# davidbau/rewriting

Hardware: NVIDIA H100
Metric: StyleGAN2-256 images/sec (higher is better)
Workload: dtype bf16x3 (3-term split bf16 operands, fp32 accumulate; fp32 in/out)

## Files before the change

### rewriting_b200/csrc/upconv_tc.cu

```cuda
#include <cstring>

#include "../../include/rewriting_b200.h"
#include "rw_common.cuh"

namespace rw {

struct UpFusedParams {
  int B, Cin, Cout, H, W;
  const float* demod;
  const float* bias;
  const float* noise;
  long long noise_bstride;
  const float* noise_w;
  const float* k4;
  const float* next_scale;
  void* next_hi;
  void* next_lo;
  float* y_out;
  int act;
  int ncg, nbands, nitems;
  long long* debug_prof;
};

namespace {

constexpr int UM = 128;
constexpr int UNC = 16;
constexpr int UN = 9 * UNC;
constexpr int UBK = 32;
constexpr int UK = 16;
constexpr int kUStages = 5;
constexpr int kUThreads = 384;
constexpr int kUTmaWarp = 8;
constexpr uint32_t kUProducerRegs = 40;
constexpr uint32_t kUConsumerRegs = 232;
constexpr int kUABytes = UM * UBK * 2;
constexpr int kUBBytes = UN * UBK * 2;
constexpr int kUStageBytes = 2 * kUABytes + 2 * kUBBytes;
constexpr int kUMailFloats = 2 * 2 * 4 * 2 * 32;
constexpr int kUOutSlotBytes = 64 * 32;
constexpr int kUOutQuarterBytes = 2 * kUOutSlotBytes;
constexpr int kUOutStageBytes = 4 * kUOutQuarterBytes;
constexpr int kUXchgFloat2 = 9 * 2 * 32;
constexpr int kUXchgBytes = 8 * kUXchgFloat2 * 8;
constexpr int kUSmemTotal =
    kUStages * kUStageBytes + kUMailFloats * 4 + kUOutStageBytes + kUXchgBytes + 512 + 256;
static_assert(kUSmemTotal <= 232448, "upconv_fused: shared memory over the per-block limit");

struct UBarriers {
  uint64_t full[kUStages];
  uint64_t empty[kUStages];
};

__device__ __forceinline__ void tma_load_5d(void* smem_dst, const CUtensorMap* m, uint64_t* bar,
                                            int32_t c0, int32_t c1, int32_t c2, int32_t c3,
                                            int32_t c4) {
  asm volatile(
      "cp.async.bulk.tensor.5d.shared::cluster.global.mbarrier::complete_tx::bytes"
      " [%0], [%1, {%3, %4, %5, %6, %7}], [%2];\n" ::"r"(smem_u32(smem_dst)),
      "l"(reinterpret_cast<uint64_t>(m)), "r"(smem_u32(bar)), "r"(c0), "r"(c1), "r"(c2), "r"(c3),
      "r"(c4)
      : "memory");
}

__device__ __forceinline__ float2 f2add(float2 a, float2 b) {
  return make_float2(__fadd_rn(a.x, b.x), __fadd_rn(a.y, b.y));
}
__device__ __forceinline__ float2 f2mul(float2 a, float2 b) {
  return make_float2(__fmul_rn(a.x, b.x), __fmul_rn(a.y, b.y));
}
__device__ __forceinline__ float2 f2fma(float2 a, float2 b, float2 c) {
  return make_float2(__fmaf_rn(a.x, b.x, c.x), __fmaf_rn(a.y, b.y, c.y));
}
__device__ __forceinline__ void mbar_wait_relaxed(uint64_t* bar, uint32_t parity) {
  uint32_t spins = 0;
  while (!mbar_try_wait(bar, parity)) {
    __nanosleep(40);
    if (++spins > RW_SPIN_LIMIT) __trap();
  }
}

__device__ __forceinline__ void sts_v4(uint32_t a, float x, float y, float z, float w) {
  asm volatile("st.shared.v4.f32 [%0], {%1, %2, %3, %4};\n" ::"r"(a), "f"(x), "f"(y), "f"(z), "f"(w)
               : "memory");
}
__device__ __forceinline__ void lds_v4(uint32_t a, float& x, float& y, float& z, float& w) {
  asm volatile("ld.shared.v4.f32 {%0, %1, %2, %3}, [%4];\n"
               : "=f"(x), "=f"(y), "=f"(z), "=f"(w)
               : "r"(a)
               : "memory");
}

constexpr int kBarPair = 3;

struct UpItem {
  int bg, band, cg;
  int y_first, y_emit, y_end;
};

__device__ __forceinline__ UpItem decode_item(int item, const UpFusedParams& p) {
  UpItem it;
  it.cg = item % p.ncg;
  const int r = item / p.ncg;
  it.band = r % p.nbands;
  it.bg = r / p.nbands;
  const int ya = 1 + (it.band * p.H) / p.nbands;
  const int yb = 1 + ((it.band + 1) * p.H) / p.nbands;
  it.y_emit = ya;
  it.y_first = ya - 2 < 0 ? 0 : ya - 2;
  it.y_end = yb;
  return it;
}

template <bool PROF, bool NCHW>
__global__ void __launch_bounds__(kUThreads, 1)
upconv_fused_kernel(const __grid_constant__ CUtensorMap map_a_hi,
                    const __grid_constant__ CUtensorMap map_a_lo,
                    const __grid_constant__ CUtensorMap map_w_hi,
                    const __grid_constant__ CUtensorMap map_w_lo,
                    const __grid_constant__ CUtensorMap map_o_hi,
                    const __grid_constant__ CUtensorMap map_o_lo, const UpFusedParams p) {
  extern __shared__ uint8_t smem_raw[];
  uint8_t* smem = reinterpret_cast<uint8_t*>((reinterpret_cast<uintptr_t>(smem_raw) + 511) &
                                             ~static_cast<uintptr_t>(511));
  float* mail = reinterpret_cast<float*>(smem + kUStages * kUStageBytes);
  uint8_t* out_stage = smem + kUStages * kUStageBytes + kUMailFloats * 4;
  float2* xchg = reinterpret_cast<float2*>(out_stage + kUOutStageBytes);
  UBarriers* bars = reinterpret_cast<UBarriers*>(out_stage + kUOutStageBytes + kUXchgBytes);

  const int warp = __shfl_sync(0xffffffffu, static_cast<int>(threadIdx.x >> 5), 0);
  const int lane = threadIdx.x & 31;
  const int kb_count = p.Cin / UBK;
  const int G = UM / p.W;

  if (warp == kUTmaWarp && lane == 0) {
    tma_prefetch_desc(&map_a_hi);
    tma_prefetch_desc(&map_a_lo);
    tma_prefetch_desc(&map_w_hi);
    tma_prefetch_desc(&map_w_lo);
    tma_prefetch_desc(&map_o_hi);
    tma_prefetch_desc(&map_o_lo);
    for (int s = 0; s < kUStages; ++s) {
      mbar_init(&bars->full[s], 1);
      mbar_init(&bars->empty[s], 2);
    }
    fence_mbar_init();
  }
  __syncthreads();

  if (warp < kUTmaWarp) {
    setmaxnreg_inc<kUConsumerRegs>();
    const int wg = warp >> 2;
    const int q = warp >> 1;
    const int h = warp & 1;
    int stage = 0;
    uint32_t phase = 0;
    const int g = lane >> 2, c = lane & 3;
    const int W = p.W;
    const int T0 = q * 32 + 4 * g;
    const int x0 = T0 & (W - 1);
    const int img_in_tile = T0 / W;
    const int Ho = 2 * p.H, Wo = 2 * W;
    const bool first_x = (x0 == 0), last_x = (x0 + 4 == W);
    const bool cross = W > 32;
    const bool mail_l = cross && g == 0 && !first_x, mail_r = cross && g == 7 && !last_x;
    float kv[4], kh[4];
    {
      const float k00 = __ldg(p.k4 + 15);
#pragma unroll
      for (int a = 0; a < 4; ++a) {
        kv[a] = __ldg(p.k4 + 15 - a * 4);
        kh[a] = __ldg(p.k4 + 15 - a) / k00;
      }
    }
    const float nw = (!NCHW || (p.noise != nullptr && p.noise_w != nullptr)) ? __ldg(p.noise_w) : 0.f;
    uint32_t step = 0;
    constexpr uint32_t kMailBufBytes = 2 * 4 * 2 * 32 * 4;
    const uint32_t mail_s = smem_u32(mail) + h * (4 * 2 * 32 * 4) + c * 32;
    const uint32_t post_r = mail_s + (q * 2 + 1) * 128, post_l = mail_s + (q * 2 + 0) * 128;
    const uint32_t read_l = mail_s + ((q - 1) * 2 + 1) * 128, read_r = mail_s + ((q + 1) * 2 + 0) * 128;
    const uint32_t slot_s = smem_u32(out_stage) + q * kUOutQuarterBytes;
    uint32_t st_addr[2];
    {
      const int m = lane >> 3, gp = lane & 7;
      const int Wm = W < 32 ? W : 32;
      const int tl = 4 * gp + m;
      const int il = tl / W;
      const int xg = ((4 * gp) & (Wm - 1)) >> 2;
#pragma unroll
      for (int xi = 0; xi < 2; ++xi) {
        uint32_t a = slot_s + (((il * 8 + 2 * m + xi) * (Wm >> 2) + xg) << 5) + (h << 4);
        a ^= ((a >> 7) & 1u) << 4;
        st_addr[xi] = a;
      }
    }
    const CUtensorMap* omap = h ? &map_o_lo : &map_o_hi;
    const uint32_t my_slot = slot_s + h * kUOutSlotBytes;
    const int o_xg = ((32 * q) & (W - 1)) >> 2;
    const int o_img = (32 * q) / W;
    long long prof_acc[16] = {0, 0, 0, 0, 0, 0, 0, 0, 0, 0, 0, 0, 0, 0, 0, 0};

    for (int item = blockIdx.x; item < p.nitems; item += gridDim.x) {
      const UpItem it = decode_item(item, p);
      const int b0 = it.bg * G;
      const int b = b0 + img_in_tile;
      const bool img_ok = b < p.B;
      const int c0 = it.cg * UNC + h * 8 + 2 * c;
      const size_t chan_o = static_cast<size_t>(img_ok ? b : 0) * p.Cout + c0;
      float2 dm = make_float2(1.f, 1.f), bs = make_float2(0.f, 0.f), ns = make_float2(1.f, 1.f);
      if (!NCHW || p.demod != nullptr) dm = __ldg(reinterpret_cast<const float2*>(p.demod + chan_o));
      if (!NCHW || (p.act && p.bias != nullptr)) bs = __ldg(reinterpret_cast<const float2*>(p.bias + c0));
      if (!NCHW) ns = __ldg(reinterpret_cast<const float2*>(p.next_scale + chan_o));
      const bool has_noise = !NCHW || (p.noise != nullptr && p.noise_w != nullptr);
      float2 c20[4], c21[4], c22[4];
      float2 w0[2][4], w1[2][4], w2[2][4];
#pragma unroll
      for (int j = 0; j < 4; ++j) {
        c20[j] = c21[j] = c22[j] = make_float2(0.f, 0.f);
        w0[0][j] = w0[1][j] = w1[0][j] = w1[1][j] = w2[0][j] = w2[1][j] = make_float2(0.f, 0.f);
      }
      const float* nrow_base = p.noise + static_cast<size_t>(img_ok ? b : 0) * p.noise_bstride + 2 * x0;
      __nv_bfloat16* out_hi = static_cast<__nv_bfloat16*>(p.next_hi);
      __nv_bfloat16* out_lo = static_cast<__nv_bfloat16*>(p.next_lo);
      const size_t img_row0 = static_cast<size_t>(img_ok ? b : 0) * (Ho + 1);

      for (int y = it.y_first; y < it.y_end; ++y, ++step) {
        const bool rows_out = (y >= it.y_emit);
        const bool emit = rows_out && img_ok;
        if (emit && c < 2 && has_noise) {
          const float* np = nrow_base + static_cast<size_t>(2 * y - 2 + c) * Wo;
          asm volatile("prefetch.global.L1 [%0];\n" ::"l"(np));
        }
        long long tq[8];
        if constexpr (PROF) tq[0] = clock64();
        float2 P[9][4];
        {
          float d[72];
          int held = -1;
          for (int kb = 0; kb < kb_count; ++kb) {
            mbar_wait(&bars->full[stage], phase);
            const uint32_t sa = smem_u32(smem + stage * kUStageBytes);
            const uint64_t da_hi = make_smem_desc(sa + wg * (kUABytes / 2), 16, 512, 2);
            const uint64_t da_lo = make_smem_desc(sa + kUABytes + wg * (kUABytes / 2), 16, 512, 2);
            const uint64_t db_hi = make_smem_desc(sa + 2 * kUABytes, 16, 512, 2);
            const uint64_t db_lo = make_smem_desc(sa + 2 * kUABytes + kUBBytes, 16, 512, 2);
            wgmma_fence();
#pragma unroll
            for (int kk = 0; kk < UBK / UK; ++kk) {
              const uint64_t adv = static_cast<uint64_t>((kk * UK * 2) >> 4);
              wgmma_m64n144<0, 0>(d, da_lo + adv, db_hi + adv, (kb | kk) != 0);
              wgmma_m64n144<0, 0>(d, da_hi + adv, db_lo + adv, 1u);
              wgmma_m64n144<0, 0>(d, da_hi + adv, db_hi + adv, 1u);
            }
            wgmma_commit();
            wgmma_wait<1>();
            if (held >= 0 && (threadIdx.x & 127) == 0) mbar_arrive(&bars->empty[held]);
            held = stage;
            if (++stage == kUStages) { stage = 0; phase ^= 1u; }
          }
          wgmma_wait<0>();
          if ((threadIdx.x & 127) == 0) mbar_arrive(&bars->empty[held]);
          if constexpr (PROF) tq[1] = clock64();
          float2* to = xchg + (warp ^ 1) * kUXchgFloat2 + lane;
#pragma unroll
          for (int t = 0; t < 9; ++t)
#pragma unroll
            for (int i = 0; i < 2; ++i)
              to[(t * 2 + i) * 32] = h ? make_float2(d[4 * t + 2 * i], d[4 * t + 2 * i + 1])
                                       : make_float2(d[4 * (9 + t) + 2 * i], d[4 * (9 + t) + 2 * i + 1]);
          named_bar_sync(kBarPair + q, 64);
          const float2* from = xchg + warp * kUXchgFloat2 + lane;
#pragma unroll
          for (int t = 0; t < 9; ++t)
#pragma unroll
            for (int i = 0; i < 2; ++i) {
              const float2 own = h ? make_float2(d[4 * (9 + t) + 2 * i], d[4 * (9 + t) + 2 * i + 1])
                                   : make_float2(d[4 * t + 2 * i], d[4 * t + 2 * i + 1]);
              const float2 other = from[(t * 2 + i) * 32];
              P[t][i] = h ? other : own;
              P[t][2 + i] = h ? own : other;
            }
          named_bar_sync(kBarPair + q, 64);
        }
        if constexpr (PROF) tq[2] = clock64();

        float2 le[2][4], ro[2][4], od[2][4];
#pragma unroll
        for (int j = 0; j < 4; ++j) {
          le[0][j] = f2add(P[0][j], c20[j]);
          od[0][j] = f2add(P[1][j], c21[j]);
          ro[0][j] = f2add(P[2][j], c22[j]);
          le[1][j] = P[3][j];
          od[1][j] = P[4][j];
          ro[1][j] = P[5][j];
          c20[j] = P[6][j];
          c21[j] = P[7][j];
          c22[j] = P[8][j];
        }
        const uint32_t mbo = (step & 1u) * kMailBufBytes;
        if (cross) {
          if (g == 7) {
            sts_v4(post_r + mbo, ro[0][3].x, ro[0][3].y, od[0][3].x, od[0][3].y);
            sts_v4(post_r + mbo + 16, ro[1][3].x, ro[1][3].y, od[1][3].x, od[1][3].y);
          }
          if (g == 0) {
            sts_v4(post_l + mbo, le[0][0].x, le[0][0].y, od[0][0].x, od[0][0].y);
            sts_v4(post_l + mbo + 16, le[1][0].x, le[1][0].y, od[1][0].x, od[1][0].y);
          }
        }
        if constexpr (PROF) tq[3] = clock64();
        float2 Lro[2], Lod[2], Rle[2], Rod[2];
#pragma unroll
        for (int r = 0; r < 2; ++r) {
          Lro[r].x = __shfl_up_sync(0xffffffffu, ro[r][3].x, 4);
          Lro[r].y = __shfl_up_sync(0xffffffffu, ro[r][3].y, 4);
          Lod[r].x = __shfl_up_sync(0xffffffffu, od[r][3].x, 4);
          Lod[r].y = __shfl_up_sync(0xffffffffu, od[r][3].y, 4);
          Rle[r].x = __shfl_down_sync(0xffffffffu, le[r][0].x, 4);
          Rle[r].y = __shfl_down_sync(0xffffffffu, le[r][0].y, 4);
          Rod[r].x = __shfl_down_sync(0xffffffffu, od[r][0].x, 4);
          Rod[r].y = __shfl_down_sync(0xffffffffu, od[r][0].y, 4);
        }
        if constexpr (PROF) tq[6] = clock64();
        const float2 kh0 = make_float2(kh[0], kh[0]), kh1 = make_float2(kh[1], kh[1]),
                     kh2 = make_float2(kh[2], kh[2]), kh3 = make_float2(kh[3], kh[3]);
        float2 hf[2][2][4];
        auto hfir = [&](int r, int j, float2 l_ro, float2 l_od, float2 r_le, float2 r_od) {
          const float2 e0 = f2add(le[r][j], l_ro);
          const float2 e1 = f2add(r_le, ro[r][j]);
          const float2 o0 = od[r][j];
          hf[r][0][j] = f2fma(kh3, e1, f2fma(kh2, o0, f2fma(kh1, e0, f2mul(kh0, l_od))));
          hf[r][1][j] = f2fma(kh3, r_od, f2fma(kh2, e1, f2fma(kh1, o0, f2mul(kh0, e0))));
        };
#pragma unroll
        for (int r = 0; r < 2; ++r) {
          hfir(r, 1, ro[r][0], od[r][0], le[r][2], od[r][2]);
          hfir(r, 2, ro[r][1], od[r][1], le[r][3], od[r][3]);
        }
        if (cross) named_bar_sync(1 + h, 128);
        if (first_x) {
#pragma unroll
          for (int r = 0; r < 2; ++r) Lro[r] = Lod[r] = make_float2(0.f, 0.f);
        } else if (mail_l) {
          lds_v4(read_l + mbo, Lro[0].x, Lro[0].y, Lod[0].x, Lod[0].y);
          lds_v4(read_l + mbo + 16, Lro[1].x, Lro[1].y, Lod[1].x, Lod[1].y);
        }
        if (last_x) {
#pragma unroll
          for (int r = 0; r < 2; ++r) Rle[r] = Rod[r] = make_float2(0.f, 0.f);
        } else if (mail_r) {
          lds_v4(read_r + mbo, Rle[0].x, Rle[0].y, Rod[0].x, Rod[0].y);
          lds_v4(read_r + mbo + 16, Rle[1].x, Rle[1].y, Rod[1].x, Rod[1].y);
        }
        if constexpr (PROF) tq[7] = clock64();
#pragma unroll
        for (int r = 0; r < 2; ++r) {
          hfir(r, 0, Lro[r], Lod[r], le[r][1], od[r][1]);
          hfir(r, 3, ro[r][2], od[r][2], Rle[r], Rod[r]);
        }
        if constexpr (PROF) tq[4] = clock64();
        if (rows_out) {
#pragma unroll
          for (int yi = 0; yi < 2; ++yi) {
            const int Y = 2 * y - 2 + yi;
            float nz[8] = {0.f, 0.f, 0.f, 0.f, 0.f, 0.f, 0.f, 0.f};
            if (has_noise) {
              const float4* np = reinterpret_cast<const float4*>(nrow_base + static_cast<size_t>(Y) * Wo);
              const float4 a4 = __ldg(np), b4 = __ldg(np + 1);
              nz[0] = a4.x; nz[1] = a4.y; nz[2] = a4.z; nz[3] = a4.w;
              nz[4] = b4.x; nz[5] = b4.y; nz[6] = b4.z; nz[7] = b4.w;
            }
            uint32_t hw[2][4], lw[2][4];
            float2 yv[2][4];
            long long te[7];
            if constexpr (PROF) te[0] = clock64();
            const float2 kv0 = make_float2(kv[0], kv[0]), kv1 = make_float2(kv[1], kv[1]),
                         kv2 = make_float2(kv[2], kv[2]), kv3 = make_float2(kv[3], kv[3]);
#pragma unroll
            for (int xi = 0; xi < 2; ++xi) {
#pragma unroll
              for (int j = 0; j < 4; ++j) {
                const float nzv = nw * nz[2 * j + xi];
                float2 v;
                if (yi == 0)
                  v = f2fma(kv3, hf[0][xi][j],
                                 f2fma(kv2, w2[xi][j], f2fma(kv1, w1[xi][j], f2mul(kv0, w0[xi][j]))));
                else
                  v = f2fma(kv3, hf[1][xi][j],
                                 f2fma(kv2, hf[0][xi][j], f2fma(kv1, w2[xi][j], f2mul(kv0, w1[xi][j]))));
                v = f2add(f2fma(v, dm, make_float2(nzv, nzv)), bs);
                if (!NCHW || p.act) {
                  const float2 t02 = f2mul(v, make_float2(0.2f, 0.2f));
                  v = f2mul(make_float2(fmaxf(v.x, t02.x), fmaxf(v.y, t02.y)),
                                 make_float2(1.4142135623730951f, 1.4142135623730951f));
                }
                if constexpr (NCHW) {
                  yv[xi][j] = v;
                } else {
                  const float2 kk = f2mul(ns, v);
                  const __nv_bfloat162 hh = __floats2bfloat162_rn(kk.x, kk.y);
                  const uint32_t hu = *reinterpret_cast<const uint32_t*>(&hh);
                  const __nv_bfloat162 ll = __floats2bfloat162_rn(
                      kk.x - __uint_as_float(hu << 16), kk.y - __uint_as_float(hu & 0xffff0000u));
                  hw[xi][j] = hu;
                  lw[xi][j] = *reinterpret_cast<const uint32_t*>(&ll);
                }
              }
            }
            if constexpr (NCHW) {
              if (img_ok) {
                float* yrow = p.y_out + ((static_cast<size_t>(b) * p.Cout + c0) * Ho + Y) * Wo + 2 * x0;
                const size_t cstride = static_cast<size_t>(Ho) * Wo;
                *reinterpret_cast<float4*>(yrow) = make_float4(yv[0][0].x, yv[1][0].x, yv[0][1].x, yv[1][1].x);
                *reinterpret_cast<float4*>(yrow + 4) = make_float4(yv[0][2].x, yv[1][2].x, yv[0][3].x, yv[1][3].x);
                *reinterpret_cast<float4*>(yrow + cstride) = make_float4(yv[0][0].y, yv[1][0].y, yv[0][1].y, yv[1][1].y);
                *reinterpret_cast<float4*>(yrow + cstride + 4) =
                    make_float4(yv[0][2].y, yv[1][2].y, yv[0][3].y, yv[1][3].y);
              }
              continue;
            }
            if constexpr (PROF) te[1] = clock64();
            if (lane == 0) tma_store_wait_read_n<0>();
            named_bar_sync(kBarPair + q, 64);
            if constexpr (PROF) te[2] = clock64();
#pragma unroll
            for (int xi = 0; xi < 2; ++xi) {
              stmatrix_x4(st_addr[xi], hw[xi]);
              stmatrix_x4(st_addr[xi] + kUOutSlotBytes, lw[xi]);
            }
            if constexpr (PROF) te[5] = clock64();
            fence_proxy_async_smem();
            if constexpr (PROF) te[6] = clock64();
            named_bar_sync(kBarPair + q, 64);
            if constexpr (PROF) te[3] = clock64();
            if (lane == 0) tma_store_5d(omap, my_slot, it.cg * UNC, o_xg, 0, Y, b0 + o_img);
            if constexpr (PROF) {
              te[4] = clock64();
#pragma unroll
              for (int i = 0; i < 4; ++i) prof_acc[8 + i] += te[i + 1] - te[i];
              prof_acc[12] += te[5] - te[2];
              prof_acc[13] += te[6] - te[5];
              prof_acc[14] += te[3] - te[6];
            }
            if (img_ok && last_x && c == 0) {
              const size_t off = ((img_row0 + Y) * (Wo + 1) + Wo) * p.Cout + it.cg * UNC + h * 8;
              *reinterpret_cast<uint4*>(out_hi + off) = make_uint4(0u, 0u, 0u, 0u);
              *reinterpret_cast<uint4*>(out_lo + off) = make_uint4(0u, 0u, 0u, 0u);
            }
          }
        }
        if (!NCHW && emit && y == p.H) {
          const size_t prow = (img_row0 + Ho) * (Wo + 1);
#pragma unroll
          for (int i = 0; i < 3; ++i) {
            if (i < 2 || (last_x && c == 3)) {
              const size_t off = (prow + 2 * x0 + 2 * c + i) * p.Cout + it.cg * UNC + h * 8;
              *reinterpret_cast<uint4*>(out_hi + off) = make_uint4(0u, 0u, 0u, 0u);
              *reinterpret_cast<uint4*>(out_lo + off) = make_uint4(0u, 0u, 0u, 0u);
            }
          }
        }
        if constexpr (PROF) {
          tq[5] = clock64();
          prof_acc[0] += tq[1] - tq[0];
          prof_acc[1] += tq[2] - tq[1];
          prof_acc[2] += tq[3] - tq[2];
          prof_acc[3] += tq[6] - tq[3];
          prof_acc[4] += tq[7] - tq[6];
          prof_acc[5] += tq[4] - tq[7];
          prof_acc[6] += tq[5] - tq[4];
          prof_acc[7] += 1;
        }
#pragma unroll
        for (int xi = 0; xi < 2; ++xi)
#pragma unroll
          for (int j = 0; j < 4; ++j) {
            w0[xi][j] = w2[xi][j];
            w1[xi][j] = hf[0][xi][j];
            w2[xi][j] = hf[1][xi][j];
          }
      }
    }
    if (!NCHW && lane == 0) tma_store_wait_all();
    if constexpr (PROF) {
      if (lane == 0 && p.debug_prof != nullptr) {
        long long* dst = p.debug_prof + (static_cast<size_t>(blockIdx.x) * 8 + warp) * 16;
#pragma unroll
        for (int i = 0; i < 16; ++i) dst[i] = prof_acc[i];
      }
    }
  } else {
    setmaxnreg_dec<kUProducerRegs>();
    if (warp != kUTmaWarp) return;
    int stage = 0;
    uint32_t phase = 0;
    const bool wide = p.W >= 32;
    const int nop = wide ? G : 4;
    const int plane = lane / nop, idx = lane % nop;
    const CUtensorMap* amap = plane ? &map_a_lo : &map_a_hi;
    const CUtensorMap* wmap = (lane & 1) ? &map_w_lo : &map_w_hi;
    const uint32_t a_off = plane * kUABytes + idx * (kUABytes / nop);
    for (int item = blockIdx.x; item < p.nitems; item += gridDim.x) {
      const UpItem it = decode_item(item, p);
      const int b0 = it.bg * G;
      const int wrow = it.cg * UN;
      for (int y = it.y_first; y < it.y_end; ++y) {
        for (int kb = 0; kb < kb_count; ++kb) {
          if (lane == 0) {
            mbar_wait_relaxed(&bars->empty[stage], phase ^ 1u);
            mbar_expect_tx(&bars->full[stage], kUStageBytes);
          }
          __syncwarp();
          uint8_t* st = smem + stage * kUStageBytes;
          if (lane < 2 * nop) {
            if (wide)
              tma_load_5d(st + a_off, amap, &bars->full[stage], kb * UBK, 0, 0, 0,
                          (b0 + idx) * (p.H + 1) + y);
            else
              tma_load_5d(st + a_off, amap, &bars->full[stage], kb * UBK, 0, b0 + idx * (32 / p.W), 0, y);
          } else if (lane >= 30) {
            tma_load_2d(st + 2 * kUABytes + (lane & 1) * kUBBytes, wmap, &bars->full[stage], kb * UBK,
                        wrow);
          }
          if (++stage == kUStages) { stage = 0; phase ^= 1u; }
        }
      }
    }
    return;
  }

}

}

static int upconv_fused_launch(const UpFusedParams& pin, const void* a_hi, const void* a_lo,
                               const void* w_hi, const void* w_lo, cudaStream_t stream) {
  UpFusedParams p = pin;
  const int W = p.W, H = p.H;
  if (W < 4 || W > UM || (W & (W - 1)) != 0 || H < 1 || p.Cin % UBK != 0 || p.Cout % UNC != 0 ||
      p.B < 1) {
    set_last_error("upconv_fused: unsupported shape B=%d Cin=%d Cout=%d H=%d W=%d", p.B, p.Cin,
                   p.Cout, H, W);
    return RW_ERR_BAD_ARG;
  }
  const int G = UM / W;
  const int nbg = (p.B + G - 1) / G;
  p.ncg = p.Cout / UNC;
  const int sms = device_sm_count();
  int best = 1;
  long long best_cost = -1;
  for (int nb = 1; nb <= 32 && H / nb >= 4; nb *= 2) {
    const long long items = static_cast<long long>(nbg) * p.ncg * nb;
    const long long waves = (items + sms - 1) / sms;
    const long long cost = waves * ((H + nb - 1) / nb + 2);
    if (best_cost < 0 || cost < best_cost) {
      best_cost = cost;
      best = nb;
    }
  }
  p.nbands = best;
  p.nitems = nbg * p.ncg * p.nbands;

  CUtensorMap ma_hi, ma_lo, mw_hi, mw_lo, mo_hi, mo_lo;
  const uint32_t Wm = W < 32 ? W : 32;
  const uint64_t kpx = static_cast<uint64_t>(p.Cin) * 2;
  const uint64_t krow = static_cast<uint64_t>(W + 1) * kpx;
  int rc;
  if (W >= 32) {
    const uint64_t dims[5] = {static_cast<uint64_t>(p.Cin), 8, 4, static_cast<uint64_t>(W / 32),
                              static_cast<uint64_t>(p.B) * (H + 1)};
    const uint64_t str[4] = {4 * kpx, kpx, 32 * kpx, krow};
    const uint32_t box[5] = {UBK, 8u, 4u, static_cast<uint32_t>(W / 32), 1u};
    if ((rc = make_tmap_nd_bf16(&ma_hi, a_hi, 5, dims, str, box, nullptr, 3))) return rc;
    if ((rc = make_tmap_nd_bf16(&ma_lo, a_lo, 5, dims, str, box, nullptr, 3))) return rc;
  } else {
    const uint64_t dims[5] = {static_cast<uint64_t>(p.Cin), static_cast<uint64_t>(W / 4),
                              static_cast<uint64_t>(p.B), 4, static_cast<uint64_t>(H + 1)};
    const uint64_t str[4] = {4 * kpx, static_cast<uint64_t>(H + 1) * krow, kpx, krow};
    const uint32_t box[5] = {UBK, static_cast<uint32_t>(W / 4), 32u / Wm, 4u, 1u};
    if ((rc = make_tmap_nd_bf16(&ma_hi, a_hi, 5, dims, str, box, nullptr, 3))) return rc;
    if ((rc = make_tmap_nd_bf16(&ma_lo, a_lo, 5, dims, str, box, nullptr, 3))) return rc;
  }
  if (p.y_out == nullptr) {
    const uint64_t Wo = 2 * static_cast<uint64_t>(W), Ho = 2 * static_cast<uint64_t>(H);
    const uint64_t px = static_cast<uint64_t>(p.Cout) * 2;
    const uint64_t od[5] = {static_cast<uint64_t>(p.Cout), Wo / 8, 8, Ho + 1, static_cast<uint64_t>(p.B)};
    const uint64_t os[4] = {8 * px, px, (Wo + 1) * px, (Ho + 1) * (Wo + 1) * px};
    const uint32_t ob[5] = {UNC, Wm / 4, 8u, 1u, 32u / Wm};
    if ((rc = make_tmap_nd_bf16(&mo_hi, p.next_hi, 5, od, os, ob, nullptr, 1))) return rc;
    if ((rc = make_tmap_nd_bf16(&mo_lo, p.next_lo, 5, od, os, ob, nullptr, 1))) return rc;
  } else {
    if ((reinterpret_cast<uintptr_t>(p.y_out) & 15u) != 0) {
      set_last_error("upconv_fused: y must be 16-byte aligned");
      return RW_ERR_BAD_ARG;
    }
    mo_hi = ma_hi;
    mo_lo = ma_lo;
  }
  const uint64_t wdims[2] = {static_cast<uint64_t>(p.Cin), static_cast<uint64_t>(p.ncg) * UN};
  const uint64_t wstr[1] = {static_cast<uint64_t>(p.Cin) * 2};
  const uint32_t wbox[2] = {UBK, UN};
  if ((rc = make_tmap_nd_bf16(&mw_hi, w_hi, 2, wdims, wstr, wbox, nullptr, 3))) return rc;
  if ((rc = make_tmap_nd_bf16(&mw_lo, w_lo, 2, wdims, wstr, wbox, nullptr, 3))) return rc;
  const int grid = p.nitems < sms ? p.nitems : sms;
  auto launch = [&](auto kernel, bool& attr_done) -> int {
    if (!attr_done) {
      int e = check_cuda(cudaFuncSetAttribute(kernel, cudaFuncAttributeMaxDynamicSharedMemorySize,
                                              kUSmemTotal),
                         "upconv_fused smem attr");
      if (e) return e;
      attr_done = true;
    }
    kernel<<<grid, kUThreads, kUSmemTotal, stream>>>(ma_hi, ma_lo, mw_hi, mw_lo, mo_hi, mo_lo, p);
    return check_cuda(cudaGetLastError(), "upconv_fused launch");
  };
  static bool attr_prof = false, attr_planes = false, attr_nchw = false;
  if (p.debug_prof != nullptr) return launch(upconv_fused_kernel<true, false>, attr_prof);
  if (p.y_out != nullptr) return launch(upconv_fused_kernel<false, true>, attr_nchw);
  return launch(upconv_fused_kernel<false, false>, attr_planes);
}

static UpFusedParams up_fused_params(int B, int Cin, int Cout, int H, int W, const float* demod,
                                     const float* kernel4x4, const float* noise,
                                     long long noise_bstride, const float* noise_w,
                                     const float* bias, const float* next_scale, void* next_hi,
                                     void* next_lo) {
  UpFusedParams p;
  memset(&p, 0, sizeof(p));
  p.B = B; p.Cin = Cin; p.Cout = Cout; p.H = H; p.W = W;
  p.demod = demod; p.bias = bias; p.noise = noise; p.noise_bstride = noise_bstride;
  p.noise_w = noise_w; p.k4 = kernel4x4; p.next_scale = next_scale;
  p.next_hi = next_hi; p.next_lo = next_lo;
  return p;
}

}

using namespace rw;

extern "C" {

int rw_modconv_up_fused(const void* kp_hi, const void* kp_lo, const void* wt_hi, const void* wt_lo,
                        const float* demod, const float* kernel4x4, const float* noise,
                        long long noise_bstride, const float* noise_w, const float* bias,
                        const float* next_scale, void* next_hi, void* next_lo, int B, int Cin,
                        int Cout, int H, int W, rw_stream_t stream) {
  if (!kp_hi || !kp_lo || !wt_hi || !wt_lo || !demod || !kernel4x4 || !noise || !noise_w || !bias ||
      !next_scale || !next_hi || !next_lo || (noise_bstride & 1)) {
    set_last_error("rw_modconv_up_fused: bad argument");
    return RW_ERR_BAD_ARG;
  }
  const UpFusedParams p = up_fused_params(B, Cin, Cout, H, W, demod, kernel4x4, noise,
                                          noise_bstride, noise_w, bias, next_scale, next_hi, next_lo);
  return upconv_fused_launch(p, kp_hi, kp_lo, wt_hi, wt_lo, stream);
}

int rw_modconv_up_fused_y(const void* kp_hi, const void* kp_lo, const void* wt_hi, const void* wt_lo,
                          const float* demod, const float* kernel4x4, const float* noise,
                          long long noise_bstride, const float* noise_w, const float* bias, int act,
                          float* y, int B, int Cin, int Cout, int H, int W, rw_stream_t stream) {
  if (!kp_hi || !kp_lo || !wt_hi || !wt_lo || !kernel4x4 || !y || (noise && (noise_bstride & 3)) ||
      ((noise != nullptr) != (noise_w != nullptr))) {
    set_last_error("rw_modconv_up_fused_y: bad argument");
    return RW_ERR_BAD_ARG;
  }
  UpFusedParams p = up_fused_params(B, Cin, Cout, H, W, demod, kernel4x4, noise, noise_bstride,
                                    noise_w, bias, nullptr, nullptr, nullptr);
  p.y_out = y;
  p.act = act;
  return upconv_fused_launch(p, kp_hi, kp_lo, wt_hi, wt_lo, stream);
}

int rw_debug_upconv_profile(const void* kp_hi, const void* kp_lo, const void* wt_hi,
                            const void* wt_lo, const float* demod, const float* kernel4x4,
                            const float* noise, long long noise_bstride, const float* noise_w,
                            const float* bias, const float* next_scale, void* next_hi, void* next_lo,
                            int B, int Cin, int Cout, int H, int W, long long* prof_out,
                            rw_stream_t stream) {
  UpFusedParams p = up_fused_params(B, Cin, Cout, H, W, demod, kernel4x4, noise, noise_bstride,
                                    noise_w, bias, next_scale, next_hi, next_lo);
  p.debug_prof = prof_out;
  return upconv_fused_launch(p, kp_hi, kp_lo, wt_hi, wt_lo, stream);
}

}
```

Measured before the change: 2067.

## Batch two output rows per TMA store and alias exchange buffer onto output slots

Each consumer pair now builds both output rows (2y-2 and 2y-1) in shared memory and issues one TMA store with a 2-row box, instead of a wait, barrier and store per row. This halves TMA stores and named barriers in the epilogue. The separate accumulator-exchange buffer is folded into the output staging slots, so a wait on pending TMA store reads is moved ahead of the exchange. W==32 gets its own single-TMA activation load mapping, and the band search now allows bands as thin as one row, which adds shared-memory reuse hazards and more registers held across the loop.

```diff
diff --git a/rewriting_b200/csrc/upconv_tc.cu b/rewriting_b200/csrc/upconv_tc.cu
--- a/rewriting_b200/csrc/upconv_tc.cu
+++ b/rewriting_b200/csrc/upconv_tc.cu
@@ -38,13 +38,15 @@
 constexpr int kUBBytes = UN * UBK * 2;
 constexpr int kUStageBytes = 2 * kUABytes + 2 * kUBBytes;
 constexpr int kUMailFloats = 2 * 2 * 4 * 2 * 32;
-constexpr int kUOutSlotBytes = 64 * 32;
-constexpr int kUOutQuarterBytes = 2 * kUOutSlotBytes;
+constexpr int kUOutRowBytes = 64 * 32;
+constexpr int kUOutSlotBytes = 2 * kUOutRowBytes;
+constexpr int kUXchgFloat2 = 9 * 2 * 32;
+constexpr int kUOutSlotStride =
+    kUXchgFloat2 * 8 > kUOutSlotBytes ? kUXchgFloat2 * 8 : kUOutSlotBytes;
+static_assert(kUOutSlotStride % 512 == 0, "upconv_fused: output slots must stay 512-byte aligned");
+constexpr int kUOutQuarterBytes = 2 * kUOutSlotStride;
 constexpr int kUOutStageBytes = 4 * kUOutQuarterBytes;
-constexpr int kUXchgFloat2 = 9 * 2 * 32;
-constexpr int kUXchgBytes = 8 * kUXchgFloat2 * 8;
-constexpr int kUSmemTotal =
-    kUStages * kUStageBytes + kUMailFloats * 4 + kUOutStageBytes + kUXchgBytes + 512 + 256;
+constexpr int kUSmemTotal = kUStages * kUStageBytes + kUMailFloats * 4 + kUOutStageBytes + 512 + 256;
 static_assert(kUSmemTotal <= 232448, "upconv_fused: shared memory over the per-block limit");
 
 struct UBarriers {
@@ -125,8 +127,7 @@
                                              ~static_cast<uintptr_t>(511));
   float* mail = reinterpret_cast<float*>(smem + kUStages * kUStageBytes);
   uint8_t* out_stage = smem + kUStages * kUStageBytes + kUMailFloats * 4;
-  float2* xchg = reinterpret_cast<float2*>(out_stage + kUOutStageBytes);
-  UBarriers* bars = reinterpret_cast<UBarriers*>(out_stage + kUOutStageBytes + kUXchgBytes);
+  UBarriers* bars = reinterpret_cast<UBarriers*>(out_stage + kUOutStageBytes);
 
   const int warp = __shfl_sync(0xffffffffu, static_cast<int>(threadIdx.x >> 5), 0);
   const int lane = threadIdx.x & 31;
@@ -180,22 +181,26 @@
     const uint32_t post_r = mail_s + (q * 2 + 1) * 128, post_l = mail_s + (q * 2 + 0) * 128;
     const uint32_t read_l = mail_s + ((q - 1) * 2 + 1) * 128, read_r = mail_s + ((q + 1) * 2 + 0) * 128;
     const uint32_t slot_s = smem_u32(out_stage) + q * kUOutQuarterBytes;
+    const int Wm = W < 32 ? W : 32;
+    const uint32_t row_bytes = 64 * Wm;
     uint32_t st_addr[2];
     {
       const int m = lane >> 3, gp = lane & 7;
-      const int Wm = W < 32 ? W : 32;
       const int tl = 4 * gp + m;
       const int il = tl / W;
       const int xg = ((4 * gp) & (Wm - 1)) >> 2;
 #pragma unroll
       for (int xi = 0; xi < 2; ++xi) {
-        uint32_t a = slot_s + (((il * 8 + 2 * m + xi) * (Wm >> 2) + xg) << 5) + (h << 4);
+        uint32_t a = slot_s + ((((il * 2) * 8 + 2 * m + xi) * (Wm >> 2) + xg) << 5) + (h << 4);
         a ^= ((a >> 7) & 1u) << 4;
         st_addr[xi] = a;
       }
     }
     const CUtensorMap* omap = h ? &map_o_lo : &map_o_hi;
-    const uint32_t my_slot = slot_s + h * kUOutSlotBytes;
+    const uint32_t my_slot = slot_s + h * kUOutSlotStride;
+    float2* const xchg_to = reinterpret_cast<float2*>(out_stage + q * kUOutQuarterBytes + h * kUOutSlotStride) + lane;
+    const float2* const xchg_from =
+        reinterpret_cast<const float2*>(out_stage + q * kUOutQuarterBytes + (h ^ 1) * kUOutSlotStride) + lane;
     const int o_xg = ((32 * q) & (W - 1)) >> 2;
     const int o_img = (32 * q) / W;
     long long prof_acc[16] = {0, 0, 0, 0, 0, 0, 0, 0, 0, 0, 0, 0, 0, 0, 0, 0};
@@ -261,7 +266,14 @@
           wgmma_wait<0>();
           if ((threadIdx.x & 127) == 0) mbar_arrive(&bars->empty[held]);
           if constexpr (PROF) tq[1] = clock64();
-          float2* to = xchg + (warp ^ 1) * kUXchgFloat2 + lane;
+          if constexpr (!NCHW) {
+            long long tw0 = 0;
+            if constexpr (PROF) tw0 = clock64();
+            if (lane == 0) tma_store_wait_read_n<0>();
+            __syncwarp();
+            if constexpr (PROF) prof_acc[9] += clock64() - tw0;
+          }
+          float2* to = xchg_to;
 #pragma unroll
           for (int t = 0; t < 9; ++t)
 #pragma unroll
@@ -269,7 +281,7 @@
               to[(t * 2 + i) * 32] = h ? make_float2(d[4 * t + 2 * i], d[4 * t + 2 * i + 1])
                                        : make_float2(d[4 * (9 + t) + 2 * i], d[4 * (9 + t) + 2 * i + 1]);
           named_bar_sync(kBarPair + q, 64);
-          const float2* from = xchg + warp * kUXchgFloat2 + lane;
+          const float2* from = xchg_from;
 #pragma unroll
           for (int t = 0; t < 9; ++t)
 #pragma unroll
@@ -360,27 +372,33 @@
         }
         if constexpr (PROF) tq[4] = clock64();
         if (rows_out) {
+          long long te[7];
+          float nz[2][8];
+#pragma unroll
+          for (int yi = 0; yi < 2; ++yi) {
+#pragma unroll
+            for (int i = 0; i < 8; ++i) nz[yi][i] = 0.f;
+            if (has_noise) {
+              const float4* np =
+                  reinterpret_cast<const float4*>(nrow_base + static_cast<size_t>(2 * y - 2 + yi) * Wo);
+              const float4 a4 = __ldg(np), b4 = __ldg(np + 1);
+              nz[yi][0] = a4.x; nz[yi][1] = a4.y; nz[yi][2] = a4.z; nz[yi][3] = a4.w;
+              nz[yi][4] = b4.x; nz[yi][5] = b4.y; nz[yi][6] = b4.z; nz[yi][7] = b4.w;
+            }
+          }
+          uint32_t hw[2][2][4], lw[2][2][4];
+          if constexpr (PROF) te[0] = clock64();
 #pragma unroll
           for (int yi = 0; yi < 2; ++yi) {
             const int Y = 2 * y - 2 + yi;
-            float nz[8] = {0.f, 0.f, 0.f, 0.f, 0.f, 0.f, 0.f, 0.f};
-            if (has_noise) {
-              const float4* np = reinterpret_cast<const float4*>(nrow_base + static_cast<size_t>(Y) * Wo);
-              const float4 a4 = __ldg(np), b4 = __ldg(np + 1);
-              nz[0] = a4.x; nz[1] = a4.y; nz[2] = a4.z; nz[3] = a4.w;
-              nz[4] = b4.x; nz[5] = b4.y; nz[6] = b4.z; nz[7] = b4.w;
-            }
-            uint32_t hw[2][4], lw[2][4];
             float2 yv[2][4];
-            long long te[7];
-            if constexpr (PROF) te[0] = clock64();
             const float2 kv0 = make_float2(kv[0], kv[0]), kv1 = make_float2(kv[1], kv[1]),
                          kv2 = make_float2(kv[2], kv[2]), kv3 = make_float2(kv[3], kv[3]);
 #pragma unroll
             for (int xi = 0; xi < 2; ++xi) {
 #pragma unroll
               for (int j = 0; j < 4; ++j) {
-                const float nzv = nw * nz[2 * j + xi];
+                const float nzv = nw * nz[yi][2 * j + xi];
                 float2 v;
                 if (yi == 0)
                   v = f2fma(kv3, hf[0][xi][j],
@@ -402,8 +420,8 @@
                   const uint32_t hu = *reinterpret_cast<const uint32_t*>(&hh);
                   const __nv_bfloat162 ll = __floats2bfloat162_rn(
                       kk.x - __uint_as_float(hu << 16), kk.y - __uint_as_float(hu & 0xffff0000u));
-                  hw[xi][j] = hu;
-                  lw[xi][j] = *reinterpret_cast<const uint32_t*>(&ll);
+                  hw[yi][xi][j] = hu;
+                  lw[yi][xi][j] = *reinterpret_cast<const uint32_t*>(&ll);
                 }
               }
             }
@@ -417,35 +435,43 @@
                 *reinterpret_cast<float4*>(yrow + cstride + 4) =
                     make_float4(yv[0][2].y, yv[1][2].y, yv[0][3].y, yv[1][3].y);
               }
-              continue;
-            }
+            }
+          }
+          if constexpr (!NCHW) {
             if constexpr (PROF) te[1] = clock64();
-            if (lane == 0) tma_store_wait_read_n<0>();
-            named_bar_sync(kBarPair + q, 64);
+#pragma unroll
+            for (int yi = 0; yi < 2; ++yi)
+#pragma unroll
+              for (int xi = 0; xi < 2; ++xi) {
+                stmatrix_x4(st_addr[xi] + yi * row_bytes, hw[yi][xi]);
+                stmatrix_x4(st_addr[xi] + yi * row_bytes + kUOutSlotStride, lw[yi][xi]);
+              }
+            if constexpr (PROF) {
+              te[5] = clock64();
+              prof_acc[8] += te[1] - te[0];
+              prof_acc[10] += te[5] - te[1];
+              prof_acc[12] += te[5] - te[1];
+            }
+            if (img_ok && last_x && c == 0) {
+#pragma unroll
+              for (int yi = 0; yi < 2; ++yi) {
+                const size_t off = ((img_row0 + 2 * y - 2 + yi) * (Wo + 1) + Wo) * p.Cout + it.cg * UNC + h * 8;
+                *reinterpret_cast<uint4*>(out_hi + off) = make_uint4(0u, 0u, 0u, 0u);
+                *reinterpret_cast<uint4*>(out_lo + off) = make_uint4(0u, 0u, 0u, 0u);
+              }
+            }
             if constexpr (PROF) te[2] = clock64();
-#pragma unroll
-            for (int xi = 0; xi < 2; ++xi) {
-              stmatrix_x4(st_addr[xi], hw[xi]);
-              stmatrix_x4(st_addr[xi] + kUOutSlotBytes, lw[xi]);
-            }
-            if constexpr (PROF) te[5] = clock64();
             fence_proxy_async_smem();
             if constexpr (PROF) te[6] = clock64();
             named_bar_sync(kBarPair + q, 64);
             if constexpr (PROF) te[3] = clock64();
-            if (lane == 0) tma_store_5d(omap, my_slot, it.cg * UNC, o_xg, 0, Y, b0 + o_img);
+            if (lane == 0) tma_store_5d(omap, my_slot, it.cg * UNC, o_xg, 0, 2 * y - 2, b0 + o_img);
             if constexpr (PROF) {
               te[4] = clock64();
-#pragma unroll
-              for (int i = 0; i < 4; ++i) prof_acc[8 + i] += te[i + 1] - te[i];
-              prof_acc[12] += te[5] - te[2];
-              prof_acc[13] += te[6] - te[5];
+              prof_acc[10] += te[3] - te[2];
+              prof_acc[11] += te[4] - te[3];
+              prof_acc[13] += te[6] - te[2];
               prof_acc[14] += te[3] - te[6];
-            }
-            if (img_ok && last_x && c == 0) {
-              const size_t off = ((img_row0 + Y) * (Wo + 1) + Wo) * p.Cout + it.cg * UNC + h * 8;
-              *reinterpret_cast<uint4*>(out_hi + off) = make_uint4(0u, 0u, 0u, 0u);
-              *reinterpret_cast<uint4*>(out_lo + off) = make_uint4(0u, 0u, 0u, 0u);
             }
           }
         }
@@ -494,8 +520,8 @@
     if (warp != kUTmaWarp) return;
     int stage = 0;
     uint32_t phase = 0;
-    const bool wide = p.W >= 32;
-    const int nop = wide ? G : 4;
+    const bool wide = p.W > 32;
+    const int nop = p.W == 32 ? 1 : wide ? G : 4;
     const int plane = lane / nop, idx = lane % nop;
     const CUtensorMap* amap = plane ? &map_a_lo : &map_a_hi;
     const CUtensorMap* wmap = (lane & 1) ? &map_w_lo : &map_w_hi;
@@ -516,6 +542,8 @@
             if (wide)
               tma_load_5d(st + a_off, amap, &bars->full[stage], kb * UBK, 0, 0, 0,
                           (b0 + idx) * (p.H + 1) + y);
+            else if (p.W == 32)
+              tma_load_5d(st + a_off, amap, &bars->full[stage], kb * UBK, 0, 0, b0, y);
             else
               tma_load_5d(st + a_off, amap, &bars->full[stage], kb * UBK, 0, b0 + idx * (32 / p.W), 0, y);
           } else if (lane >= 30) {
@@ -549,7 +577,7 @@
   const int sms = device_sm_count();
   int best = 1;
   long long best_cost = -1;
-  for (int nb = 1; nb <= 32 && H / nb >= 4; nb *= 2) {
+  for (int nb = 1; nb <= 32 && nb <= H; nb *= 2) {
     const long long items = static_cast<long long>(nbg) * p.ncg * nb;
     const long long waves = (items + sms - 1) / sms;
     const long long cost = waves * ((H + nb - 1) / nb + 2);
@@ -566,7 +594,14 @@
   const uint64_t kpx = static_cast<uint64_t>(p.Cin) * 2;
   const uint64_t krow = static_cast<uint64_t>(W + 1) * kpx;
   int rc;
-  if (W >= 32) {
+  if (W == 32) {
+    const uint64_t dims[5] = {static_cast<uint64_t>(p.Cin), 8, 4, static_cast<uint64_t>(p.B),
+                              static_cast<uint64_t>(H + 1)};
+    const uint64_t str[4] = {4 * kpx, kpx, static_cast<uint64_t>(H + 1) * krow, krow};
+    const uint32_t box[5] = {UBK, 8u, 4u, static_cast<uint32_t>(G), 1u};
+    if ((rc = make_tmap_nd_bf16(&ma_hi, a_hi, 5, dims, str, box, nullptr, 3))) return rc;
+    if ((rc = make_tmap_nd_bf16(&ma_lo, a_lo, 5, dims, str, box, nullptr, 3))) return rc;
+  } else if (W > 32) {
     const uint64_t dims[5] = {static_cast<uint64_t>(p.Cin), 8, 4, static_cast<uint64_t>(W / 32),
                               static_cast<uint64_t>(p.B) * (H + 1)};
     const uint64_t str[4] = {4 * kpx, kpx, 32 * kpx, krow};
@@ -586,7 +621,7 @@
     const uint64_t px = static_cast<uint64_t>(p.Cout) * 2;
     const uint64_t od[5] = {static_cast<uint64_t>(p.Cout), Wo / 8, 8, Ho + 1, static_cast<uint64_t>(p.B)};
     const uint64_t os[4] = {8 * px, px, (Wo + 1) * px, (Ho + 1) * (Wo + 1) * px};
-    const uint32_t ob[5] = {UNC, Wm / 4, 8u, 1u, 32u / Wm};
+    const uint32_t ob[5] = {UNC, Wm / 4, 8u, 2u, 32u / Wm};
     if ((rc = make_tmap_nd_bf16(&mo_hi, p.next_hi, 5, od, os, ob, nullptr, 1))) return rc;
     if ((rc = make_tmap_nd_bf16(&mo_lo, p.next_lo, 5, od, os, ob, nullptr, 1))) return rc;
   } else {
```

Result: faster. 2092 (median of 6 runs) (+1.2%).

## Software-pipeline next row's WGMMA GEMM under the current row's FIR epilogue

Applied to the files above, without the earlier changes.

Restructures the consumer loop so the tensor-core GEMM for the next row is issued in chunks (pump) interleaved with the current row's horizontal FIR, mailbox exchange and output stores. Accumulators are spilled to a shared-memory tile that also carries the vertical-tap overlap, replacing the register carry and the separate exchange buffer. Pipeline stages drop from 5 to 4 to make room for the tile. This aims to hide epilogue latency behind MMA work, at the cost of extra shared-memory traffic, register pressure from holding 72 accumulators alongside epilogue state, and a shallower TMA pipeline.

```diff
diff --git a/rewriting_b200/csrc/upconv_tc.cu b/rewriting_b200/csrc/upconv_tc.cu
--- a/rewriting_b200/csrc/upconv_tc.cu
+++ b/rewriting_b200/csrc/upconv_tc.cu
@@ -29,7 +29,7 @@
 constexpr int UN = 9 * UNC;
 constexpr int UBK = 32;
 constexpr int UK = 16;
-constexpr int kUStages = 5;
+constexpr int kUStages = 4;
 constexpr int kUThreads = 384;
 constexpr int kUTmaWarp = 8;
 constexpr uint32_t kUProducerRegs = 40;
@@ -39,12 +39,11 @@
 constexpr int kUStageBytes = 2 * kUABytes + 2 * kUBBytes;
 constexpr int kUMailFloats = 2 * 2 * 4 * 2 * 32;
 constexpr int kUOutSlotBytes = 64 * 32;
-constexpr int kUOutQuarterBytes = 2 * kUOutSlotBytes;
-constexpr int kUOutStageBytes = 4 * kUOutQuarterBytes;
-constexpr int kUXchgFloat2 = 9 * 2 * 32;
-constexpr int kUXchgBytes = 8 * kUXchgFloat2 * 8;
+constexpr int kUTileQuarterBytes = 2 * 9 * 2 * 32 * 16;
+constexpr int kUTileBytes = 4 * kUTileQuarterBytes;
+static_assert(2 * kUOutSlotBytes <= 6 * 2 * 32 * 16, "upconv_fused: staging slots over taps 0..5");
 constexpr int kUSmemTotal =
-    kUStages * kUStageBytes + kUMailFloats * 4 + kUOutStageBytes + kUXchgBytes + 512 + 256;
+    kUStages * kUStageBytes + kUMailFloats * 4 + kUTileBytes + 512 + 256;
 static_assert(kUSmemTotal <= 232448, "upconv_fused: shared memory over the per-block limit");
 
 struct UBarriers {
@@ -124,9 +123,9 @@
   uint8_t* smem = reinterpret_cast<uint8_t*>((reinterpret_cast<uintptr_t>(smem_raw) + 511) &
                                              ~static_cast<uintptr_t>(511));
   float* mail = reinterpret_cast<float*>(smem + kUStages * kUStageBytes);
-  uint8_t* out_stage = smem + kUStages * kUStageBytes + kUMailFloats * 4;
-  float2* xchg = reinterpret_cast<float2*>(out_stage + kUOutStageBytes);
-  UBarriers* bars = reinterpret_cast<UBarriers*>(out_stage + kUOutStageBytes + kUXchgBytes);
+  float4* tile = reinterpret_cast<float4*>(smem + kUStages * kUStageBytes + kUMailFloats * 4);
+  UBarriers* bars = reinterpret_cast<UBarriers*>(smem + kUStages * kUStageBytes + kUMailFloats * 4 +
+                                                 kUTileBytes);
 
   const int warp = __shfl_sync(0xffffffffu, static_cast<int>(threadIdx.x >> 5), 0);
   const int lane = threadIdx.x & 31;
@@ -179,7 +178,7 @@
     const uint32_t mail_s = smem_u32(mail) + h * (4 * 2 * 32 * 4) + c * 32;
     const uint32_t post_r = mail_s + (q * 2 + 1) * 128, post_l = mail_s + (q * 2 + 0) * 128;
     const uint32_t read_l = mail_s + ((q - 1) * 2 + 1) * 128, read_r = mail_s + ((q + 1) * 2 + 0) * 128;
-    const uint32_t slot_s = smem_u32(out_stage) + q * kUOutQuarterBytes;
+    const uint32_t slot_s = smem_u32(tile) + q * kUTileQuarterBytes;
     uint32_t st_addr[2];
     {
       const int m = lane >> 3, gp = lane & 7;
@@ -199,6 +198,63 @@
     const int o_xg = ((32 * q) & (W - 1)) >> 2;
     const int o_img = (32 * q) / W;
     long long prof_acc[16] = {0, 0, 0, 0, 0, 0, 0, 0, 0, 0, 0, 0, 0, 0, 0, 0};
+
+    float d[72];
+    int held = -1;
+    int kn = 0, kn_end = 0;
+    auto pump = [&]() {
+      if (kn < kn_end) {
+        mbar_wait(&bars->full[stage], phase);
+        const uint32_t sa = smem_u32(smem + stage * kUStageBytes);
+        const uint64_t da_hi = make_smem_desc(sa + wg * (kUABytes / 2), 16, 512, 2);
+        const uint64_t da_lo = make_smem_desc(sa + kUABytes + wg * (kUABytes / 2), 16, 512, 2);
+        const uint64_t db_hi = make_smem_desc(sa + 2 * kUABytes, 16, 512, 2);
+        const uint64_t db_lo = make_smem_desc(sa + 2 * kUABytes + kUBBytes, 16, 512, 2);
+        wgmma_fence();
+#pragma unroll
+        for (int kk = 0; kk < UBK / UK; ++kk) {
+          const uint64_t adv = static_cast<uint64_t>((kk * UK * 2) >> 4);
+          wgmma_m64n144<0, 0>(d, da_lo + adv, db_hi + adv, (kn | kk) != 0);
+          wgmma_m64n144<0, 0>(d, da_hi + adv, db_lo + adv, 1u);
+          wgmma_m64n144<0, 0>(d, da_hi + adv, db_hi + adv, 1u);
+        }
+        wgmma_commit();
+        wgmma_wait<1>();
+        if (held >= 0 && (threadIdx.x & 127) == 0) mbar_arrive(&bars->empty[held]);
+        held = stage;
+        if (++stage == kUStages) { stage = 0; phase ^= 1u; }
+        ++kn;
+      }
+    };
+    float4* const tile_w = tile + (q * 2 * 9 * 2 + h) * 32 + lane;
+    const uint32_t tile_rs = smem_u32(tile + (q * 2 + h) * 9 * 2 * 32 + lane);
+    auto finish = [&](bool carry) {
+      while (kn < kn_end) pump();
+      wgmma_wait<0>();
+      if (held >= 0 && (threadIdx.x & 127) == 0) mbar_arrive(&bars->empty[held]);
+      held = -1;
+      kn = 0;
+      if (kn_end == 0) return;
+      if (!NCHW && lane == 0) tma_store_wait_read_n<0>();
+      named_bar_sync(kBarPair + q, 64);
+#pragma unroll
+      for (int hc = 0; hc < 2; ++hc)
+#pragma unroll
+        for (int t = 0; t < 9; ++t) {
+          float4 v = make_float4(d[4 * (9 * hc + t)], d[4 * (9 * hc + t) + 1], d[4 * (9 * hc + t) + 2],
+                                 d[4 * (9 * hc + t) + 3]);
+          float4* dst = tile_w + (hc * 9 + t) * 64;
+          if (t < 3 && carry) {
+            const float4 o = dst[6 * 64];
+            v = make_float4(__fadd_rn(v.x, o.x), __fadd_rn(v.y, o.y), __fadd_rn(v.z, o.z),
+                            __fadd_rn(v.w, o.w));
+          }
+          *dst = v;
+        }
+      named_bar_sync(kBarPair + q, 64);
+    };
+    kn_end = kb_count;
+    finish(false);
 
     for (int item = blockIdx.x; item < p.nitems; item += gridDim.x) {
       const UpItem it = decode_item(item, p);
@@ -212,13 +268,10 @@
       if (!NCHW || (p.act && p.bias != nullptr)) bs = __ldg(reinterpret_cast<const float2*>(p.bias + c0));
       if (!NCHW) ns = __ldg(reinterpret_cast<const float2*>(p.next_scale + chan_o));
       const bool has_noise = !NCHW || (p.noise != nullptr && p.noise_w != nullptr);
-      float2 c20[4], c21[4], c22[4];
       float2 w0[2][4], w1[2][4], w2[2][4];
 #pragma unroll
-      for (int j = 0; j < 4; ++j) {
-        c20[j] = c21[j] = c22[j] = make_float2(0.f, 0.f);
+      for (int j = 0; j < 4; ++j)
         w0[0][j] = w0[1][j] = w1[0][j] = w1[1][j] = w2[0][j] = w2[1][j] = make_float2(0.f, 0.f);
-      }
       const float* nrow_base = p.noise + static_cast<size_t>(img_ok ? b : 0) * p.noise_bstride + 2 * x0;
       __nv_bfloat16* out_hi = static_cast<__nv_bfloat16*>(p.next_hi);
       __nv_bfloat16* out_lo = static_cast<__nv_bfloat16*>(p.next_lo);
@@ -231,112 +284,57 @@
           const float* np = nrow_base + static_cast<size_t>(2 * y - 2 + c) * Wo;
           asm volatile("prefetch.global.L1 [%0];\n" ::"l"(np));
         }
+        const bool last_row = (y + 1 == it.y_end);
+        kn_end = (!last_row || item + static_cast<int>(gridDim.x) < p.nitems) ? kb_count : 0;
         long long tq[8];
         if constexpr (PROF) tq[0] = clock64();
-        float2 P[9][4];
-        {
-          float d[72];
-          int held = -1;
-          for (int kb = 0; kb < kb_count; ++kb) {
-            mbar_wait(&bars->full[stage], phase);
-            const uint32_t sa = smem_u32(smem + stage * kUStageBytes);
-            const uint64_t da_hi = make_smem_desc(sa + wg * (kUABytes / 2), 16, 512, 2);
-            const uint64_t da_lo = make_smem_desc(sa + kUABytes + wg * (kUABytes / 2), 16, 512, 2);
-            const uint64_t db_hi = make_smem_desc(sa + 2 * kUABytes, 16, 512, 2);
-            const uint64_t db_lo = make_smem_desc(sa + 2 * kUABytes + kUBBytes, 16, 512, 2);
-            wgmma_fence();
-#pragma unroll
-            for (int kk = 0; kk < UBK / UK; ++kk) {
-              const uint64_t adv = static_cast<uint64_t>((kk * UK * 2) >> 4);
-              wgmma_m64n144<0, 0>(d, da_lo + adv, db_hi + adv, (kb | kk) != 0);
-              wgmma_m64n144<0, 0>(d, da_hi + adv, db_lo + adv, 1u);
-              wgmma_m64n144<0, 0>(d, da_hi + adv, db_hi + adv, 1u);
-            }
-            wgmma_commit();
-            wgmma_wait<1>();
-            if (held >= 0 && (threadIdx.x & 127) == 0) mbar_arrive(&bars->empty[held]);
-            held = stage;
-            if (++stage == kUStages) { stage = 0; phase ^= 1u; }
+        float2 le[4], od[4], ro[4];
+        auto load_row = [&](int r) {
+#pragma unroll
+          for (int jp = 0; jp < 2; ++jp) {
+            float4 a, o, e;
+            lds_v4(tile_rs + ((3 * r + 0) * 2 + jp) * 512, a.x, a.y, a.z, a.w);
+            lds_v4(tile_rs + ((3 * r + 1) * 2 + jp) * 512, o.x, o.y, o.z, o.w);
+            lds_v4(tile_rs + ((3 * r + 2) * 2 + jp) * 512, e.x, e.y, e.z, e.w);
+            le[2 * jp] = make_float2(a.x, a.y);
+            le[2 * jp + 1] = make_float2(a.z, a.w);
+            od[2 * jp] = make_float2(o.x, o.y);
+            od[2 * jp + 1] = make_float2(o.z, o.w);
+            ro[2 * jp] = make_float2(e.x, e.y);
+            ro[2 * jp + 1] = make_float2(e.z, e.w);
           }
-          wgmma_wait<0>();
-          if ((threadIdx.x & 127) == 0) mbar_arrive(&bars->empty[held]);
-          if constexpr (PROF) tq[1] = clock64();
-          float2* to = xchg + (warp ^ 1) * kUXchgFloat2 + lane;
-#pragma unroll
-          for (int t = 0; t < 9; ++t)
-#pragma unroll
-            for (int i = 0; i < 2; ++i)
-              to[(t * 2 + i) * 32] = h ? make_float2(d[4 * t + 2 * i], d[4 * t + 2 * i + 1])
-                                       : make_float2(d[4 * (9 + t) + 2 * i], d[4 * (9 + t) + 2 * i + 1]);
-          named_bar_sync(kBarPair + q, 64);
-          const float2* from = xchg + warp * kUXchgFloat2 + lane;
-#pragma unroll
-          for (int t = 0; t < 9; ++t)
-#pragma unroll
-            for (int i = 0; i < 2; ++i) {
-              const float2 own = h ? make_float2(d[4 * (9 + t) + 2 * i], d[4 * (9 + t) + 2 * i + 1])
-                                   : make_float2(d[4 * t + 2 * i], d[4 * t + 2 * i + 1]);
-              const float2 other = from[(t * 2 + i) * 32];
-              P[t][i] = h ? other : own;
-              P[t][2 + i] = h ? own : other;
-            }
-          named_bar_sync(kBarPair + q, 64);
-        }
-        if constexpr (PROF) tq[2] = clock64();
-
-        float2 le[2][4], ro[2][4], od[2][4];
-#pragma unroll
-        for (int j = 0; j < 4; ++j) {
-          le[0][j] = f2add(P[0][j], c20[j]);
-          od[0][j] = f2add(P[1][j], c21[j]);
-          ro[0][j] = f2add(P[2][j], c22[j]);
-          le[1][j] = P[3][j];
-          od[1][j] = P[4][j];
-          ro[1][j] = P[5][j];
-          c20[j] = P[6][j];
-          c21[j] = P[7][j];
-          c22[j] = P[8][j];
-        }
-        const uint32_t mbo = (step & 1u) * kMailBufBytes;
-        if (cross) {
-          if (g == 7) {
-            sts_v4(post_r + mbo, ro[0][3].x, ro[0][3].y, od[0][3].x, od[0][3].y);
-            sts_v4(post_r + mbo + 16, ro[1][3].x, ro[1][3].y, od[1][3].x, od[1][3].y);
-          }
-          if (g == 0) {
-            sts_v4(post_l + mbo, le[0][0].x, le[0][0].y, od[0][0].x, od[0][0].y);
-            sts_v4(post_l + mbo + 16, le[1][0].x, le[1][0].y, od[1][0].x, od[1][0].y);
-          }
-        }
-        if constexpr (PROF) tq[3] = clock64();
-        float2 Lro[2], Lod[2], Rle[2], Rod[2];
-#pragma unroll
-        for (int r = 0; r < 2; ++r) {
-          Lro[r].x = __shfl_up_sync(0xffffffffu, ro[r][3].x, 4);
-          Lro[r].y = __shfl_up_sync(0xffffffffu, ro[r][3].y, 4);
-          Lod[r].x = __shfl_up_sync(0xffffffffu, od[r][3].x, 4);
-          Lod[r].y = __shfl_up_sync(0xffffffffu, od[r][3].y, 4);
-          Rle[r].x = __shfl_down_sync(0xffffffffu, le[r][0].x, 4);
-          Rle[r].y = __shfl_down_sync(0xffffffffu, le[r][0].y, 4);
-          Rod[r].x = __shfl_down_sync(0xffffffffu, od[r][0].x, 4);
-          Rod[r].y = __shfl_down_sync(0xffffffffu, od[r][0].y, 4);
-        }
-        if constexpr (PROF) tq[6] = clock64();
+        };
         const float2 kh0 = make_float2(kh[0], kh[0]), kh1 = make_float2(kh[1], kh[1]),
                      kh2 = make_float2(kh[2], kh[2]), kh3 = make_float2(kh[3], kh[3]);
         float2 hf[2][2][4];
         auto hfir = [&](int r, int j, float2 l_ro, float2 l_od, float2 r_le, float2 r_od) {
-          const float2 e0 = f2add(le[r][j], l_ro);
-          const float2 e1 = f2add(r_le, ro[r][j]);
-          const float2 o0 = od[r][j];
+          const float2 e0 = f2add(le[j], l_ro);
+          const float2 e1 = f2add(r_le, ro[j]);
+          const float2 o0 = od[j];
           hf[r][0][j] = f2fma(kh3, e1, f2fma(kh2, o0, f2fma(kh1, e0, f2mul(kh0, l_od))));
           hf[r][1][j] = f2fma(kh3, r_od, f2fma(kh2, e1, f2fma(kh1, o0, f2mul(kh0, e0))));
         };
+        float2 Lro[2], Lod[2], Rle[2], Rod[2];
+        const uint32_t mbo = (step & 1u) * kMailBufBytes;
 #pragma unroll
         for (int r = 0; r < 2; ++r) {
-          hfir(r, 1, ro[r][0], od[r][0], le[r][2], od[r][2]);
-          hfir(r, 2, ro[r][1], od[r][1], le[r][3], od[r][3]);
-        }
+          load_row(r);
+          if (r == 0) pump();
+          if (cross && g == 7) sts_v4(post_r + mbo + 16 * r, ro[3].x, ro[3].y, od[3].x, od[3].y);
+          if (cross && g == 0) sts_v4(post_l + mbo + 16 * r, le[0].x, le[0].y, od[0].x, od[0].y);
+          Lro[r].x = __shfl_up_sync(0xffffffffu, ro[3].x, 4);
+          Lro[r].y = __shfl_up_sync(0xffffffffu, ro[3].y, 4);
+          Lod[r].x = __shfl_up_sync(0xffffffffu, od[3].x, 4);
+          Lod[r].y = __shfl_up_sync(0xffffffffu, od[3].y, 4);
+          Rle[r].x = __shfl_down_sync(0xffffffffu, le[0].x, 4);
+          Rle[r].y = __shfl_down_sync(0xffffffffu, le[0].y, 4);
+          Rod[r].x = __shfl_down_sync(0xffffffffu, od[0].x, 4);
+          Rod[r].y = __shfl_down_sync(0xffffffffu, od[0].y, 4);
+          hfir(r, 1, ro[0], od[0], le[2], od[2]);
+          hfir(r, 2, ro[1], od[1], le[3], od[3]);
+        }
+        pump();
+        if constexpr (PROF) tq[2] = clock64();
         if (cross) named_bar_sync(1 + h, 128);
         if (first_x) {
 #pragma unroll
@@ -352,12 +350,14 @@
           lds_v4(read_r + mbo, Rle[0].x, Rle[0].y, Rod[0].x, Rod[0].y);
           lds_v4(read_r + mbo + 16, Rle[1].x, Rle[1].y, Rod[1].x, Rod[1].y);
         }
-        if constexpr (PROF) tq[7] = clock64();
+        if constexpr (PROF) tq[3] = clock64();
 #pragma unroll
         for (int r = 0; r < 2; ++r) {
-          hfir(r, 0, Lro[r], Lod[r], le[r][1], od[r][1]);
-          hfir(r, 3, ro[r][2], od[r][2], Rle[r], Rod[r]);
-        }
+          load_row(r);
+          hfir(r, 0, Lro[r], Lod[r], le[1], od[1]);
+          hfir(r, 3, ro[2], od[2], Rle[r], Rod[r]);
+        }
+        pump();
         if constexpr (PROF) tq[4] = clock64();
         if (rows_out) {
 #pragma unroll
@@ -407,6 +407,7 @@
                 }
               }
             }
+            pump();
             if constexpr (NCHW) {
               if (img_ok) {
                 float* yrow = p.y_out + ((static_cast<size_t>(b) * p.Cout + c0) * Ho + Y) * Wo + 2 * x0;
@@ -434,6 +435,7 @@
             named_bar_sync(kBarPair + q, 64);
             if constexpr (PROF) te[3] = clock64();
             if (lane == 0) tma_store_5d(omap, my_slot, it.cg * UNC, o_xg, 0, Y, b0 + o_img);
+            pump();
             if constexpr (PROF) {
               te[4] = clock64();
 #pragma unroll
@@ -460,17 +462,6 @@
             }
           }
         }
-        if constexpr (PROF) {
-          tq[5] = clock64();
-          prof_acc[0] += tq[1] - tq[0];
-          prof_acc[1] += tq[2] - tq[1];
-          prof_acc[2] += tq[3] - tq[2];
-          prof_acc[3] += tq[6] - tq[3];
-          prof_acc[4] += tq[7] - tq[6];
-          prof_acc[5] += tq[4] - tq[7];
-          prof_acc[6] += tq[5] - tq[4];
-          prof_acc[7] += 1;
-        }
 #pragma unroll
         for (int xi = 0; xi < 2; ++xi)
 #pragma unroll
@@ -479,6 +470,20 @@
             w1[xi][j] = hf[0][xi][j];
             w2[xi][j] = hf[1][xi][j];
           }
+        if constexpr (PROF) {
+          tq[5] = clock64();
+          prof_acc[15] += kn;
+        }
+        finish(!last_row);
+        if constexpr (PROF) {
+          tq[1] = clock64();
+          prof_acc[0] += tq[1] - tq[5];
+          prof_acc[1] += tq[2] - tq[0];
+          prof_acc[2] += tq[3] - tq[2];
+          prof_acc[3] += tq[4] - tq[3];
+          prof_acc[6] += tq[5] - tq[4];
+          prof_acc[7] += 1;
+        }
       }
     }
     if (!NCHW && lane == 0) tma_store_wait_all();
```

Result: no change. 2078 before, 2079 after (median of 6 runs) (+0.0%).
